# tmbdev/clstm

Measured on AMD Instinct MI355X. Metric: text-line images/sec (fwd+bwd+CTC), 100-unit BiLSTM H=48 T~200, higher is better.
Workload: dtype f32 (operand-exact split): forward, recurrences, CTC, decode in f32 arithmetic; the backward weight-gradient / softmax-backward products take their f32 operands split EXACTLY into three bf16 terms each (x1 + x2 + x3 = x) and sum the six bf16-MFMA products of weight >= 2^-16 in f32 -- what is dropped

## Files before the change

clstm_amd/abi.py:

```python
import ctypes as C
import os

import numpy as np

_HERE = os.path.dirname(os.path.abspath(__file__))
MAX_LAYERS = 4


class NetDesc(C.Structure):
    _fields_ = [("nlayers", C.c_int), ("unidirectional", C.c_int), ("ninput", C.c_int),
                ("nhidden", C.c_int * MAX_LAYERS), ("nclasses", C.c_int)]


class ClstmError(RuntimeError):
    pass


def default_lib_path():
    variant = os.environ.get("CLSTM_HIP_VARIANT", "")
    name = "libclstm_hip_%s.so" % variant if variant else "libclstm_hip.so"
    return os.environ.get("CLSTM_HIP_LIB", os.path.join(_HERE, "lib", name))


_P, _I, _F = C.c_void_p, C.c_int, C.c_float
# ... 91 lines not shown
    "clstm_comm_rank": [_P],
    "clstm_comm_size": [_P],
    "clstm_comm_peer_active": [_P],
    "clstm_comm_peer_capacity": [_P, _P],
    "clstm_allreduce_flat": [_P, _P, C.c_longlong],
    "clstm_net_set_comm": [_P, _P],
    "clstm_net_replica_check": [_P],
    "clstm_net_set_training": [_P, _I],
    "clstm_net_set_overlap": [_P, _I],
    "clstm_net_get_overlap": [_P, _P],
    "clstm_net_set_strict_f32": [_P, _I],
    "clstm_net_overlap_stats": [_P, _P, _P],
    "clstm_debug_lane_ops": [_P],
    "clstm_debug_ctc_cycles": [_P],
    "clstm_debug_gemm": [_I, _P, _P, _P, _I, _I, _I, _I],
    "clstm_debug_path_count": [_I, _P],
    "clstm_debug_set_option": [C.c_char_p, _I],
    "clstm_debug_set_device_error": [_I, _I],
    "clstm_debug_wide_plan": [_P, _P],
    "clstm_debug_net_holds": [_P, _P],
    "clstm_debug_narrow_plan": [_P, _P],
    "clstm_debug_product_plan": [_P, _P],
    "clstm_debug_ctc_plan": [_I, _P, _P, _P, _I, _P, _P],
}
_VALUE_RETURN = {"clstm_net_nparams_for", "clstm_net_nparams", "clstm_abi_version", "clstm_comm_rank", "clstm_comm_size", "clstm_comm_peer_active"}
EXPORTED_SYMBOLS = sorted(list(_SIGS) + ["clstm_last_error", "clstm_abi_version"])
_LATE = {"clstm_debug_net_holds", "clstm_debug_wide_plan", "clstm_debug_narrow_plan", "clstm_debug_product_plan", "clstm_debug_ctc_plan"}


class Lib:

    def __init__(self, path=None):
        path = path or default_lib_path()
        if not os.path.exists(path):
            raise ClstmError(
                "HIP extension not built: %s is missing (no CPU fallback exists; build it with "
                "`make -C clstm_amd/csrc` or __graft_entry__.build())" % path)
        self.path = path
        if os.path.basename(path).startswith("libclstm_hip"):
            try:
                import torch
            except ImportError:
                pass
        self.dll = C.CDLL(path)
        self.dll.clstm_last_error.restype = C.c_char_p
        self.dll.clstm_last_error.argtypes = []
        self.dll.clstm_abi_version.restype = C.c_int
        for name, args in _SIGS.items():
            if (name in _LATE or os.environ.get("CLSTM_ABI_LAX")) and not hasattr(self.dll, name):
                continue
# ... 44 lines not shown
```

clstm_amd/csrc/abi.inc:

```
using namespace clstm;
struct clstm_net {
  std::unique_ptr<size_t> dev_bytes;
  Net net;
  CtcWorkspace ctc;
  DecodeWorkspace dec;
  ScoreWorkspace score;
  BeamWorkspace beam;
};

#define EW(kernel, len, ...) \
  CLSTM_LAUNCH(kernel, dim3(nblocks(len)), dim3(256), 0, g_stream, __VA_ARGS__); check_launch();

struct clstm_charlm { CharLm lm; };
struct clstm_normalizer {
  std::unique_ptr<size_t> dev_bytes;
  Normalizer nz;
};
extern "C" {

const char* clstm_last_error(void) { return g_err.c_str(); }
int clstm_abi_version(void) { return 1; }
int clstm_set_stream(void* s) { g_stream = (hipStream_t)s; return 0; }
int clstm_synchronize(void) { ABI_BEGIN HIPCHECK(hipStreamSynchronize(g_stream)); check_device_errors(); ABI_END }

// ... 768 lines not shown
  static_assert(sizeof(NarrowShape) == 30 * sizeof(int) && sizeof(NarrowPlan) == 11 * sizeof(int), "include/clstm_abi.h documents the int layout");
  NarrowShape h;
  memcpy(&h, shape, sizeof(h));
  REQUIRE(h.pass >= NP_FWD_SAVE && h.pass <= NP_BWD && h.no > 0 && h.ndir >= 1 && h.bs > 0 && h.ncu >= 0, "bad shape");
  const NarrowPlan p = narrow_plan(h);
  memcpy(plan, &p, sizeof(p));
  ABI_END
}
int clstm_debug_product_plan(const int* shape, int* plan) {
  ABI_BEGIN
  REQUIRE(shape && plan, "null argument");
  static_assert(sizeof(ProductShape) == 35 * sizeof(int) && sizeof(ProductPlan) == 39 * sizeof(int), "include/clstm_abi.h documents the int layout");
  ProductShape h;
  memcpy(&h, shape, sizeof(h));
  REQUIRE(h.pass >= PP_FWD && h.pass <= PP_BWD && h.no > 0 && h.ni > 0 && h.ndir >= 1 && h.N > 0 && h.nclasses >= 2 && h.ncu >= 0, "bad shape");
  const ProductPlan p = product_plan(h);
  memcpy(plan, &p, sizeof(p));
  ABI_END
}
int clstm_debug_ctc_plan(int nc, const int* line_off_h, const int* states_h, const int* state_off_h, int bs, int* batch_plan_h,
                         int* line_plan_h) {
  ABI_BEGIN
  describe_ctc_plan(nc, line_off_h, states_h, state_off_h, bs, batch_plan_h, line_plan_h);
  ABI_END
}
int clstm_debug_lane_ops(float* out) {
  ABI_BEGIN
  CLSTM_LAUNCH(k_debug_lane_ops, dim3(1), dim3(64), 0, g_stream, out);
  check_launch();
  ABI_END
}
int clstm_debug_gemm(int mode, const float* A, const float* B, float* Cm, int R, int Cn, int K, int nsplit) {
  ABI_BEGIN
  static thread_local DevBuf<float>* part = nullptr;
  const int sq = gemm_bf16_big(R, Cn) ? GB2_BT : GEMM_BT, kk = gemm_tile256(R, Cn) ? 256 : GB2_BT;
  if (mode == 0) gemm_f32<GEMM_KC, GEMM_MC>(g_stream, gemm_kc(A, K, R, 0), gemm_mc(B, Cn, K, 0), StorePlain{Cm, Cn}, R, Cn, K);
  else if (mode == 1) gemm_f32<GEMM_KC, GEMM_KC>(g_stream, gemm_kc(A, K, R, 0), gemm_kc(B, K, Cn, 0), StorePlain{Cm, Cn}, R, Cn, K);
  else if (mode == 2) {
    if (!part) part = new DevBuf<float>();
    if (nsplit < 1) nsplit = 1;
    part->reserve((size_t)nsplit * R * Cn);
    gemm_f32<GEMM_MC, GEMM_MC>(g_stream, gemm_mc(A, R, K, 0), gemm_mc(B, Cn, K, 0), StorePartial{part->p, R, Cn}, R, Cn, K, nsplit);
    CLSTM_LAUNCH(k_reduce_scatter, dim3(nblocks((size_t)R * Cn)), dim3(256), 0, g_stream,
                 (ReduceDesc{part->p, nullptr, 0LL, nsplit, 1, R, Cn, Cn}), (ReduceDesc{}), Cm, (int*)nullptr, 0, (UpdateFuse{}));
  } else if (mode == 10) gemm_bf16<GEMM_KC, GEMM_MC>(g_stream, gemm_kc(A, K, R, 0), gemm_mc(B, Cn, K, 0), StorePlain{Cm, Cn}, R, Cn, K, sq);
  else if (mode == 11) gemm_bf16<GEMM_KC, GEMM_KC>(g_stream, gemm_kc(A, K, R, 0), gemm_kc(B, K, Cn, 0), StorePlain{Cm, Cn}, R, Cn, K, sq);
// ... 47 lines not shown
```

clstm_amd/csrc/ctc.h:

```cpp
#pragma once
#include <type_traits>
#include "devintrin.h"
#define CR_FN DEVFN
#include "cr_math.h"

namespace clstm {

constexpr int CTC_THREADS = 512;
constexpr int CTC_GROUP = 256;
constexpr int CTC_RMAX = 8;
constexpr int CTC_SMAX_LDS = CTC_GROUP * CTC_RMAX;
constexpr int CTC_MLP = 8;
constexpr int CTC_MLPT = 20;
constexpr int CTC_MAX_TILE = 256;
#ifndef CLSTM_CTC_PD
#define CLSTM_CTC_PD 8
#endif
constexpr int CTC_PD = CLSTM_CTC_PD;
constexpr int CTC_PREG = 34;
constexpr int CTC_NB = 12;
constexpr int CTC_CLANE = 32;
constexpr int CTC_CCACHE = 26;

struct CtcLine { long long lat_off; int b, off, T, soff, S, nu; };
struct CtcArgs {
  const CtcLine* lines;
  const float* P;
  float* Dz;
  float* aligned;
  const int* states;
  float* lat;
  const double* tables;
  int nc;
  int ncp;
  int tile;
  int smax;
  long long* prof;
  int float_logadd;
};

struct CtcLds {
  int tables, part, tot, rowbuf, etile, asum, states, lists, ucol, ucls, ccol, vx, red, dump, words;
};
inline __host__ __device__ CtcLds ctc_lds_layout(int tile, int ncp, int smax) {
  CtcLds l;
  int o = 0;
  l.tables = o; o += CTC_TABLE_WORDS;
  l.part = o;   o += 2 * 512;
  l.tot = o;    o += 2 * smax;
  o = (o + 3) & ~3;
  l.rowbuf = o; o += tile * ncp;
  l.etile = o;  o += tile * (smax | 1);
  l.asum = o;   o += tile;
  l.states = o; o += smax;
  l.lists = o;  o += smax;
  l.ucol = o;   o += smax;
  l.ucls = o;   o += smax;
  l.ccol = o;   o += ncp <= CTC_THREADS + 1 ? ncp : 0;
  l.vx = o;     o += 2 * 2 * (CTC_GROUP + 2);
  l.red = o;    o += 64;
  l.dump = o;   o += 2;
  l.words = o;
  return l;
}
inline __host__ __device__ int ctc_region_words(const CtcLds& l, int tile) { return l.asum + tile - l.rowbuf; }

struct CtcBatchPlan { int tile, smax, ncp, smem; };
inline CtcBatchPlan ctc_batch_plan(int nc, int smax_lines, int tmax) {
  CtcBatchPlan p;
  p.smax = smax_lines < 1 ? 1 : (smax_lines > CTC_SMAX_LDS ? CTC_SMAX_LDS : smax_lines);
  if (tmax < 1) tmax = 1;
  p.ncp = nc | 1;
  const long fixed = (long)ctc_lds_layout(0, p.ncp, p.smax).words * (long)sizeof(float);
  int tile = (int)((160 * 1024 - fixed) / (long)((p.ncp + (p.smax | 1) + 1) * sizeof(float)));
  if (tile > CTC_MAX_TILE) tile = CTC_MAX_TILE;
  if (tile > tmax) tile = tmax;
  p.tile = tile;
  p.smem = (int)((size_t)ctc_lds_layout(tile < 1 ? 1 : tile, p.ncp, p.smax).words * sizeof(float));
  return p;
}
enum CtcForm { CTC_FORM_SHORT = 0, CTC_FORM_TILED = 1, CTC_FORM_HUGE = 2, CTC_FORM_NONE = 3 };
enum CtcRec { CTC_REC_WAVE = 0, CTC_REC_PAIR = 1, CTC_REC_RM2 = 2, CTC_REC_RM8 = 3, CTC_REC_ROUNDS = 4 };
struct CtcLinePlan {
  int form, rec;
  int flat, lds_lat, lanemap;
  int flat_stage, c_in_regs, d_per_state, ntiles;
};
inline __host__ __device__ CtcLinePlan ctc_line_plan(int T, int S, int nu, int nc, int ncp, int tile, int cap) {
  CtcLinePlan p{CTC_FORM_NONE, 0, 0, 0, 0, 0, 0, 0, 0};
  if (T <= 0 || S <= 0) return p;
  const int nub_mk = ((S + 1) / 2 < nc ? (S + 1) / 2 : nc) | 1;
  const int nub = (nu | 1) > nub_mk ? (nu | 1) : nub_mk;
  const bool short_line = T <= CTC_THREADS && (long)T * (ncp + nub) <= cap && (long)T * ((S | 1) + nub) <= cap &&
                          S <= CTC_THREADS && T * S <= CTC_THREADS * CTC_CCACHE && nc <= CTC_THREADS;
  p.form = short_line ? CTC_FORM_SHORT : (S > CTC_SMAX_LDS ? CTC_FORM_HUGE : CTC_FORM_TILED);
  p.rec = S <= 64 ? CTC_REC_WAVE : S <= 128 ? CTC_REC_PAIR : S > CTC_SMAX_LDS ? CTC_REC_ROUNDS
        : (S + CTC_GROUP - 1) / CTC_GROUP <= 2 ? CTC_REC_RM2 : CTC_REC_RM8;
  if (short_line) {
    p.flat = ncp == nc && T * nc <= CTC_PREG * CTC_THREADS;
    p.lds_lat = S <= 64 && 2 * T * S <= cap;
    p.lanemap = S <= 64 && T <= (CTC_THREADS / 64) * CTC_CLANE;
  } else {
    p.flat_stage = ncp == nc;
    p.c_in_regs = (long)T * S <= CTC_THREADS * CTC_CCACHE;
    p.d_per_state = S > CTC_THREADS;
    p.ntiles = (T + tile - 1) / tile;
  }
  return p;
}
inline __host__ __device__ int ctc_scores_behind(int T, int S, int ncp) { return 2 * T * S > T * ncp ? 2 * T * S : T * ncp; }
inline __host__ __device__ bool ctc_scores_in_lds(const CtcLinePlan& p, int T, int S, int ncp, int nu, int cap) {
  return p.lds_lat && ctc_scores_behind(T, S, ncp) + T * (nu | 1) <= cap;
}

DEVFN float ctc_softplus_float(float d) {
  const float L2E_HI = 1.44269502162933349609375f, L2E_LO = 1.92596299112661746e-8f;
  const float t = d * L2E_HI;
  const float r = fmaf(d, L2E_LO, fmaf(d, L2E_HI, -t));
  const float e2 = fast_exp2(t);
  const float ef = fmaf(e2 * 0.693147182464599609375f, r, e2);
  const float sf = ef + 1.0f;
  return fast_log2(sf) * 0.693147182464599609375f;
}
template <bool FLA = false>
DEVFN float ctc_log_add(float x, float y, const CrTables tb) {
  const float d = x - y;
  float lg;
  if constexpr (FLA) lg = ctc_softplus_float(fminf(fmaxf(d, -10.0f), 10.0f)) + y;
  else lg = cr_softplusf(d, tb) + y;
  return fabsf(d) > 10.0f ? fmaxf(x, y) : lg;
}
DEVFN float ctc_limexp(float x) {
  const float xc = fminf(fmaxf(x, -30.0f), 30.0f);
  const float L2E_HI = 1.44269502162933349609375f, L2E_LO = 1.92596299112661746e-8f;
  const float t = xc * L2E_HI;
  const float r = fmaf(xc, L2E_LO, fmaf(xc, L2E_HI, -t));
// ... 175 lines not shown
template <bool FLA = false>
DEVFN void ctc_lattice_huge(const float* lm, float* al, float* be, const CrTables tb, const int T, const int S) {
  const int tid = threadIdx.x;
  const int grp = tid >> 8, u = tid & (CTC_GROUP - 1);
  const bool rev = grp == 1;
  const size_t latbytes = (size_t)T * S * 4;
  const BufF32 lmb = make_buf(lm, latbytes), outb = make_buf(rev ? be : al, latbytes);
  auto loff = [&](int i, int j) -> unsigned {
    return (unsigned)(rev ? (size_t)(T - 1 - i) * S + (S - 1 - j) : (size_t)i * S + j) * 4u;
  };
  __syncthreads();
  for (int i = 0; i < T; i++) {
    for (int j = u; j < S; j += CTC_GROUP) {
      const float lmv = buf_load(lmb, loff(i, j));
      const float vj = i == 0 ? (float)(-5.0 * j) : buf_load_wt(outb, loff(i - 1, j));
      const float w = j == 0 ? (float)(-5.0 * i) : (i == 0 ? (float)(-5.0 * (j - 1)) : buf_load_wt(outb, loff(i - 1, j - 1)));
      buf_store_wt(outb, loff(i, j), ctc_log_add<FLA>(vj + lmv, w + lmv, tb));
    }
    drain_vmem();
    __syncthreads();
  }
}

#define CTC_STAMP(k) do { if (a.prof && b == 0 && threadIdx.x == 0) a.prof[k] = dev_clock(); } while (0)
constexpr int CTC_TREG = (CTC_TABLE_DOUBLES + CTC_THREADS - 1) / CTC_THREADS;

template <bool FLA>
DEVFN void ctc_short_line(const CtcArgs& a, float* lds, const CtcLds& L, const CrTables tb, const int b, float* lm,
                          const int off, const int T, const int S, const double (&treg)[CTC_TREG],
                          const float (&preg)[CTC_PREG], const CtcLinePlan& pl) {
  const int tid = threadIdx.x, lane = tid & 63, wave = wave_uniform(tid >> 6);
  const int nc = a.nc, ncp = a.ncp;
  double* part = reinterpret_cast<double*>(lds + L.part);
  double* tot = reinterpret_cast<double*>(lds + L.tot);
  float* rowbuf = lds + L.rowbuf;
  float* etile = rowbuf;
  const int cap = ctc_region_words(L, a.tile);
  const bool flat = pl.flat;
  int* stl = reinterpret_cast<int*>(lds + L.states);
  int* lists = reinterpret_cast<int*>(lds + L.lists);
  int* ucol = reinterpret_cast<int*>(lds + L.ucol);
  int* ucls = reinterpret_cast<int*>(lds + L.ucls);
  int* ccol = reinterpret_cast<int*>(lds + L.ccol);
  float* red = lds + L.red;
  int* wcnt = reinterpret_cast<int*>(red + 16);
  float* dump = lds + L.dump;
  float* al = lm + (size_t)T * S;
  float* be = al + (size_t)T * S;
  const int TS = T * S, sp = S | 1;
  const size_t latbytes = (size_t)TS * 4;
  const BufF32 pb = make_buf(a.P + (size_t)off * nc, (size_t)T * nc * 4);

  const int npost = T * nc;

  int* firstof = reinterpret_cast<int*>(rowbuf);
// ... 20 lines not shown
  for (int w = 0; w < CTC_THREADS / 64; w++) {
    const int cP = wcnt[w * 4], cB = wcnt[w * 4 + 1], cL = wcnt[w * 4 + 2], cR = wcnt[w * 4 + 3];
    const bool pre = w < wave;
    bP += pre ? cP : 0; bB += pre ? cB : 0; bL += pre ? cL : 0; bR += pre ? cR : 0;
    nu += cP; nb += cB; nf += cL;
  }
  const int nr = S - nb - nf, nup = nu | 1;
  if (tid < nc) {
    const int r = bP + __builtin_popcountll(mP & below);
    ccol[tid] = pres ? r : -1;
    if (pres) ucls[r] = tid;
  }
  if (isblank) lists[bB + __builtin_popcountll(mB & below)] = tid;
  if (islab) lists[nb + bL + __builtin_popcountll(mL & below)] = tid;
  if (isrep) lists[nb + nf + bR + __builtin_popcountll(mR & below)] = tid;
  __syncthreads();
  if (live) ucol[tid] = ccol[sc];
  CTC_STAMP(12);
  const bool lds_lat = pl.lds_lat;
  const bool lm_lds = ctc_scores_in_lds(pl, T, S, ncp, nu, cap);
  float* lmu = rowbuf + (lm_lds ? ctc_scores_behind(T, S, ncp) : T * ncp);
  float pw[CTC_NB];
  {
    const int n = T * nu;
    const int dq = CTC_THREADS / nu, dr = CTC_THREADS - dq * nu;
    int tq = tid / nu, uq = tid - tq * nu;
#pragma unroll
    for (int u = 0; u < CTC_NB; u++) {
      const bool in = tid + u * CTC_THREADS < n;
      pw[u] = buf_load(pb, in ? (unsigned)(tq * nc + ucls[in ? uq : 0]) * 4u : BUF_OOB);
      tq += dq; uq += dr;
      if (uq >= nu) { uq -= nu; tq++; }
    }
  }
  {
    double* tabs = reinterpret_cast<double*>(lds + L.tables);
#pragma unroll
    for (int k = 0; k < CTC_TREG; k++)
      if (tid + k * CTC_THREADS < CTC_TABLE_DOUBLES) tabs[tid + k * CTC_THREADS] = treg[k];
  }

  if (flat) {
#pragma unroll
    for (int k = 0; k < CTC_PREG; k++) {
      const int i = tid + k * CTC_THREADS;
      float* w = i < npost ? &rowbuf[i] : dump;
      *w = fmaxf(1e-5f, preg[k]);
    }
  } else {
// ... 75 lines not shown
#pragma unroll
        for (int u = 0; u < 8; u++) {
          const int t = t0 + u * (CTC_THREADS / 64);
          buf_store(lmw, (sok && t < T) ? (unsigned)(t * S + st) * 4u : BUF_OOB, x[u]);
        }
      }
    }
  }
  CTC_STAMP(1);

  float* all = rowbuf;
  float* bel = rowbuf + TS;
  if (lm_lds) ctc_lattice<true, true, FLA>(lm, all, bel, lds + L.vx, dump, tb, T, S, pl.rec, lmu, nup, ucol);
  else if (lds_lat) ctc_lattice<true, false, FLA>(lm, all, bel, lds + L.vx, dump, tb, T, S, pl.rec);
  else ctc_lattice<false, false, FLA, CTC_REC_RM2>(lm, al, be, lds + L.vx, dump, tb, T, S, pl.rec);
  const BufF32 dzb = make_buf(a.Dz + (size_t)off * nc, (size_t)T * nc * 4);
  const BufF32 agb = make_buf(a.aligned ? a.aligned + (size_t)off * nc : a.Dz, a.aligned ? (size_t)T * nc * 4 : 0);
  const bool one_wave = pl.rec == CTC_REC_WAVE;
  if (!one_wave || (wave & 2)) {
    const int w0 = !one_wave ? wave : (wave & 1) + ((wave >> 2) << 1), nw = !one_wave ? CTC_THREADS / 64 : 4;
    for (int cb = 0; cb < nc; cb += 64) {
      const int c = cb + lane;
      const bool absent = c < nc && ccol[c < nc ? c : 0] < 0;
      for (int t0 = w0; t0 < T; t0 += 8 * nw) {
        float x[8];
        unsigned ofs[8];
#pragma unroll
        for (int u = 0; u < 8; u++) {
          const int t = t0 + u * nw;
          ofs[u] = (absent && t < T) ? (unsigned)(t * nc + c) * 4u : BUF_OOB;
          x[u] = buf_load(pb, ofs[u]);
        }
#pragma unroll
        for (int u = 0; u < 8; u++) {
          buf_store(agb, ofs[u], 0.0f);
          buf_store(dzb, ofs[u], 0.0f - x[u]);
        }
      }
    }
  }
  __syncthreads();
  CTC_STAMP(2);

  const bool lanemap = pl.lanemap;
  if (lanemap) {
    const BufF32 alb = make_buf(al, latbytes), beb = make_buf(be, latbytes);
    const bool sok = lane < S;
    const int sl = sok ? lane : 0;
    float bo[CTC_CLANE];
    float mx = -3.0e38f;
    auto load_cells = [&](auto lds_tag) {
      constexpr bool LL = decltype(lds_tag)::value;
#pragma unroll
// ... 33 lines not shown
    for (int g = 0; g < CTC_CLANE / 4; g++) {
      if (wave + 32 * g < T) {
#pragma unroll
        for (int u = 0; u < 4; u++) {
          const int k = 4 * g + u, t = wave + 8 * k;
          const float e = ctc_limexp(bo[k] - mx);
          bo[k] = e;
          acc += (t < T) ? (double)e : 0.0;
        }
      }
    }
    CTC_STAMP(3);
    if (sok) part[wave * S + lane] = acc;
    __syncthreads();
    CTC_STAMP(8);
    if (tid < S) {
      double sum = 0.0;
      for (int k = 0; k < CTC_THREADS / 64; k++) sum += part[k * S + tid];
      tot[tid] = 1.0 / fmax(1e-9, sum);
    }
    __syncthreads();
    CTC_STAMP(9);
    const double it = tot[sl];
#pragma unroll
    for (int g = 0; g < CTC_CLANE / 4; g++) {
      if (wave + 32 * g < T) {
#pragma unroll
        for (int u = 0; u < 4; u++) {
          const int k = 4 * g + u, t = wave + 8 * k;
          float* w = (sok && t < T) ? &etile[t * sp + lane] : dump;
          *w = (float)((double)bo[k] * it);
        }
      }
    }
    __syncthreads();
    CTC_STAMP(4);
  } else {
  {
    const BufF32 alb = make_buf(al, latbytes), beb = make_buf(be, latbytes);
    float bo[CTC_CCACHE];
    float mx = -3.0e38f;
    if (lds_lat) {
#pragma unroll
      for (int k = 0; k < CTC_CCACHE; k++) {
        const int i = tid + k * CTC_THREADS;
        const int ic = i < TS ? i : 0;
        bo[k] = i < TS ? all[ic] + bel[ic] : -3.0e38f;
        mx = fmaxf(mx, bo[k]);
      }
    } else {
#pragma unroll
      for (int k = 0; k < CTC_CCACHE; k++) {
        const int i = tid + k * CTC_THREADS;
// ... 46 lines not shown
    if (act) part[q * S + st] = acc;
    __syncthreads();
    CTC_STAMP(8);
    if (tid < S) {
      double sum = 0.0;
      for (int k = 0; k < Q; k++) sum += part[k * S + tid];
      tot[tid] = 1.0 / fmax(1e-9, sum);
    }
    __syncthreads();
    CTC_STAMP(9);
  }
  CTC_STAMP(4);
  }

  float* rowc = rowbuf + T * sp;
  auto project = [&](auto pre_tag) {
    constexpr bool PRE = decltype(pre_tag)::value;
    if (wave >= 4) {
      for (int f0 = 0; f0 < nf; f0 += 64) {
        const bool fok = f0 + lane < nf;
        const int st = lists[nb + (fok ? f0 + lane : 0)];
        const int col = ucol[st];
        const double it = PRE ? 1.0 : tot[st];
        int t0 = wave - 4;
        for (; t0 + 28 < T; t0 += 4 * 8) {
          float x[8];
#pragma unroll
          for (int u = 0; u < 8; u++) x[u] = etile[(t0 + 4 * u) * sp + st];
#pragma unroll
          for (int u = 0; u < 8; u++) {
            float* w = fok ? &rowc[(t0 + 4 * u) * nup + col] : dump;
            *w = PRE ? x[u] : (float)((double)x[u] * it);
          }
        }
        if (t0 < T) {
          float x[8];
#pragma unroll
          for (int u = 0; u < 8; u++) { const int t = t0 + 4 * u; x[u] = etile[(t < T ? t : T - 1) * sp + st]; }
#pragma unroll
          for (int u = 0; u < 8; u++) {
            const int t = t0 + 4 * u;
            float* w = (fok && t < T) ? &rowc[t * nup + col] : dump;
            *w = PRE ? x[u] : (float)((double)x[u] * it);
          }
        }
      }
    } else {
      for (int t = tid; t < T; t += 256) {
        const float* e = etile + t * sp;
        double blank = 0.0;
        int i0 = 0;
        for (; i0 + 8 <= nb; i0 += 8) {
          float x[8];
          double it[8];
#pragma unroll
          for (int u = 0; u < 8; u++) {
            const int st = lists[i0 + u];
            x[u] = e[st];
            it[u] = PRE ? 1.0 : tot[st];
          }
#pragma unroll
          for (int u = 0; u < 8; u++) blank += PRE ? (double)x[u] : (double)(float)((double)x[u] * it[u]);
        }
        if (i0 < nb) {
          float x[8];
          double it[8];
#pragma unroll
          for (int u = 0; u < 8; u++) {
            const int st = lists[i0 + u < nb ? i0 + u : 0];
            x[u] = e[st];
            it[u] = PRE ? 1.0 : tot[st];
          }
#pragma unroll
          for (int u = 0; u < 8; u++) blank += (i0 + u < nb) ? (PRE ? (double)x[u] : (double)(float)((double)x[u] * it[u])) : 0.0;
        }
        part[t] = blank;
      }
    }
  };
  if (lanemap) project(std::true_type{}); else project(std::false_type{});
  __syncthreads();
  CTC_STAMP(10);
  for (int t = tid; t < T; t += CTC_THREADS) {
    float* row = rowc + t * nup;
    const float* e = etile + t * sp;
    for (int i = 0; i < nr; i++) {
      const int st = lists[nb + nf + i];
      row[ucol[st]] += lanemap ? e[st] : (float)((double)e[st] * tot[st]);
    }
    if (nb > 0) row[ccol[0]] = (float)part[t];
    double total = 0.0;
    int u0 = 0;
    for (; u0 + 8 <= nu; u0 += 8) {
      float x[8];
#pragma unroll
      for (int u = 0; u < 8; u++) x[u] = row[u0 + u];
#pragma unroll
      for (int u = 0; u < 8; u++) total += (double)x[u];
    }
    if (u0 < nu) {
      float x[8];
#pragma unroll
      for (int u = 0; u < 8; u++) x[u] = row[u0 + u < nu ? u0 + u : 0];
#pragma unroll
      for (int u = 0; u < 8; u++) total += (u0 + u < nu) ? (double)x[u] : 0.0;
    }
    part[t] = 1.0 / fmax(total, 1e-9);
  }
  __syncthreads();
  CTC_STAMP(11);
  {
    const int n = T * nu;
    const int dq = CTC_THREADS / nu, dr = CTC_THREADS - dq * nu;
    int tq = tid / nu, uq = tid - tq * nu;
    for (int i0 = tid; i0 < n; i0 += CTC_NB * CTC_THREADS) {
      float p[CTC_NB], av[CTC_NB];
      unsigned ofs[CTC_NB];
#pragma unroll
      for (int u = 0; u < CTC_NB; u++) {
        const bool in = i0 + u * CTC_THREADS < n;
        const int tc = in ? tq : 0, uc = in ? uq : 0;
        ofs[u] = in ? (unsigned)(tc * nc + ucls[uc]) * 4u : BUF_OOB;
        av[u] = (float)((double)rowc[tc * nup + uc] * part[tc]);
        tq += dq; uq += dr;
        if (uq >= nu) { uq -= nu; tq++; }
      }
      if (i0 == tid) {
#pragma unroll
        for (int u = 0; u < CTC_NB; u++) p[u] = pw[u];
      } else {
#pragma unroll
        for (int u = 0; u < CTC_NB; u++) p[u] = buf_load(pb, ofs[u]);
      }
#pragma unroll
      for (int u = 0; u < CTC_NB; u++) {
        buf_store(agb, ofs[u], av[u]);
        buf_store(dzb, ofs[u], av[u] - p[u]);
      }
    }
  }
  CTC_STAMP(5);
}

template <bool FLA>
__global__ __launch_bounds__(CTC_THREADS) void ctc_align_kernel(CtcArgs a) {
  float* lds = dyn_smem<float>();
  const CtcLds L = ctc_lds_layout(a.tile, a.ncp, a.smax);
  double* tabs = reinterpret_cast<double*>(lds + L.tables);
  double* part = reinterpret_cast<double*>(lds + L.part);
  double* tot = reinterpret_cast<double*>(lds + L.tot);
  float* rowbuf = lds + L.rowbuf;
  float* etile = lds + L.etile;
  float* asum = lds + L.asum;
  int* stl = reinterpret_cast<int*>(lds + L.states);
  float* vx = lds + L.vx;
  float* red = lds + L.red;
  const CrTables tb{tabs, tabs + 32, tabs + 96, tabs + 160};
  const int tid = threadIdx.x, lane = tid & 63, wave = wave_uniform(tid >> 6);
  const CtcLine ln = a.lines[blockIdx.x];
  const int b = ln.b;
  const int nc = a.nc, ncp = a.ncp, TT = a.tile;
  const int off = ln.off, T = ln.T;
  const int soff = ln.soff, S = ln.S;
  const CtcLinePlan pl = ctc_line_plan(T, S, ln.nu, nc, ncp, TT, ctc_region_words(L, TT));
  if (pl.form == CTC_FORM_NONE) return;
  const float* P = a.P + (size_t)off * nc;
  float* Dz = a.Dz + (size_t)off * nc;
  float* lm = a.lat + ln.lat_off;
  float* al = lm + (size_t)T * S;
  float* be = al + (size_t)T * S;
  CTC_STAMP(0);
  const bool short_line = pl.form == CTC_FORM_SHORT;
  const int st0 = a.states[soff + (tid < S ? tid : 0)];
  double treg[CTC_TREG];
#pragma unroll
  for (int k = 0; k < CTC_TREG; k++) {
    const int i = tid + k * CTC_THREADS;
    treg[k] = a.tables[i < CTC_TABLE_DOUBLES ? i : CTC_TABLE_DOUBLES - 1];
  }
  if (short_line) {
    const BufF32 pb = make_buf(P, (size_t)T * nc * 4);
    float preg[CTC_PREG];
    if (pl.flat) {
#pragma unroll
      for (int k = 0; k < CTC_PREG; k++) preg[k] = buf_load(pb, (unsigned)(tid + k * CTC_THREADS) * 4u);
    }
    if (tid < S) stl[tid] = st0;
    for (int s = tid + CTC_THREADS; s < S; s += CTC_THREADS) stl[s] = a.states[soff + s];
    __syncthreads();
    ctc_short_line<FLA>(a, lds, L, tb, b, lm, off, T, S, treg, preg, pl);
    return;
  }
  const bool huge = pl.form == CTC_FORM_HUGE;
  const int* stg = a.states + soff;
  double* totg = reinterpret_cast<double*>(lm + (((size_t)3 * T * S + 1) & ~(size_t)1));
  if (!huge) {
    if (tid < S) stl[tid] = st0;
    for (int s = tid + CTC_THREADS; s < S; s += CTC_THREADS) stl[s] = a.states[soff + s];
  }
  auto state_at = [&](int s) -> int { return huge ? stg[s] : stl[s]; };
  int* lists = reinterpret_cast<int*>(lds + L.lists);
  int nblank = 0;
  if (!huge) {
    __syncthreads();
    int* cnt = reinterpret_cast<int*>(red + 32);
    if (wave == 0) {
      int nb = 0;
      for (int s0 = 0; s0 < S; s0 += 64) nb += __builtin_popcountll(wave_ballot(s0 + lane < S && stl[s0 + lane < S ? s0 + lane : 0] == 0));
      int ib = 0, il = nb;
      const unsigned long long below = (1ull << lane) - 1ull;
      for (int s0 = 0; s0 < S; s0 += 64) {
        const bool in = s0 + lane < S;
        const bool isb = in && stl[in ? s0 + lane : 0] == 0;
// ... 328 lines not shown
```

clstm_amd/csrc/ctc_run.inc:

```
static thread_local long long* g_last_ctc_prof = nullptr;
struct CtcWorkspace {
  CtcArgs pending{};
  size_t pending_smem = 0;
  int pending_bs = 0;
  PinnedRing ring;
  DevBuf<long long> prof;
  DevBuf<double> tables;
  DevBuf<char> meta;
  DevBuf<float> lat;
  std::vector<int> nu, seen;
};
static void upload_ctc_tables(DevBuf<double>& tables) {
  if (tables.p) return;
  tables.reserve(CTC_TABLE_DOUBLES);
  std::vector<double> tb(CTC_TABLE_DOUBLES);
  for (int i = 0; i < 32; i++) tb[i] = CTC_EXP2_32[i];
  for (int i = 0; i < 64; i++) { tb[32 + i] = CTC_LOG_INVC[i]; tb[96 + i] = CTC_LOG_LOGC[i]; }
  for (int k = 0; k < 2 * CTC_SP_KMAX + 1; k++)
    for (int c = 0; c < 4; c++) tb[160 + 4 * k + c] = CTC_SOFTPLUS[k][c];
  HIPCHECK(hipMemcpy(tables.p, tb.data(), CTC_TABLE_DOUBLES * sizeof(double), hipMemcpyHostToDevice));
}
static void launch_ctc_align(const CtcWorkspace& w, hipStream_t s) {
  if (!w.pending.float_logadd) CLSTM_LAUNCH(ctc_align_kernel<false>, dim3(w.pending_bs), dim3(CTC_THREADS), w.pending_smem, s, w.pending);
  else CLSTM_LAUNCH(ctc_align_kernel<true>, dim3(w.pending_bs), dim3(CTC_THREADS), w.pending_smem, s, w.pending);
  check_launch();
}
static void expand_transcripts(const int* labels_h, const int* L_h, int n, std::vector<int>& states, std::vector<int>& soff) {
  soff.assign(n + 1, 0);
  int lpos = 0;
  for (int b = 0; b < n; b++) {
    const int L = L_h[b];
    REQUIRE(L >= 0, "negative transcript length");
    states.resize(soff[b] + 2 * L + 1);
    clstm_mktargets(states.data() + soff[b], labels_h + lpos, L);
    for (int i = 0; i < L; i++) REQUIRE(labels_h[lpos + i] != 0, "transcript contains the blank class (Codec::encode asserts c != 0, clstm.cc:232)");
    lpos += L;
    soff[b + 1] = soff[b] + 2 * L + 1;
  }
}
static void check_target_classes(int nc, const int* states_h, int ns) {
  for (int i = 0; i < ns; i++) REQUIRE(states_h[i] >= 0 && states_h[i] < nc, "target class out of range");
}
static CtcBatchPlan ctc_minibatch_plan(int nc, const int* line_off_h, const int* state_off_h, int bs) {
  int smax = 1, tmax = 1;
  for (int b = 0; b < bs; b++) {
    smax = std::max(smax, state_off_h[b + 1] - state_off_h[b]);
    tmax = std::max(tmax, line_off_h[b + 1] - line_off_h[b]);
  }
  const CtcBatchPlan bp = ctc_batch_plan(nc, smax, tmax);
  REQUIRE(bp.tile >= 1, "too many classes / target states for the CTC row tile");
  REQUIRE(bp.smem <= 160 * 1024, "CTC LDS carve exceeds 160 KiB");
  return bp;
}
static void ctc_distinct_classes(int nc, const int* states_h, const int* state_off_h, int bs, std::vector<int>& nu, std::vector<int>& seen) {
  nu.assign(bs, 0);
  seen.assign(nc, -1);
  for (int b = 0; b < bs; b++)
    for (int i = state_off_h[b]; i < state_off_h[b + 1]; i++)
      if (seen[states_h[i]] != b) { seen[states_h[i]] = b; nu[b]++; }
}
constexpr int CTC_PLAN_INTS = 13;
static void describe_ctc_plan(int nc, const int* line_off_h, const int* states_h, const int* state_off_h, int bs, int* batch_plan_h,
                              int* line_plan_h) {
  REQUIRE(bs > 0 && nc >= 1 && line_off_h && states_h && state_off_h && batch_plan_h && line_plan_h, "empty batch / null argument");
  for (int b = 0; b < bs; b++)
    REQUIRE(line_off_h[b + 1] >= line_off_h[b] && state_off_h[b + 1] >= state_off_h[b], "bad offsets");
  check_target_classes(nc, states_h, state_off_h[bs]);
  const CtcBatchPlan bp = ctc_minibatch_plan(nc, line_off_h, state_off_h, bs);
  batch_plan_h[0] = bp.tile; batch_plan_h[1] = bp.smax; batch_plan_h[2] = bp.ncp; batch_plan_h[3] = bp.smem;
  const int cap = ctc_region_words(ctc_lds_layout(bp.tile, bp.ncp, bp.smax), bp.tile);
  std::vector<int> nus, seen;
  ctc_distinct_classes(nc, states_h, state_off_h, bs, nus, seen);
// ... 28 lines not shown
  {
    char* stage = (char*)w.ring.acquire(nln + nst);
    std::vector<int> order(bs);
    for (int b = 0; b < bs; b++) order[b] = b;
    std::stable_sort(order.begin(), order.end(), [&](int x, int y) { return lo[x + 1] - lo[x] > lo[y + 1] - lo[y]; });
    CtcLine* ln = (CtcLine*)stage;
    for (int i = 0; i < bs; i++) {
      const int b = order[i];
      ln[i] = CtcLine{lo[b], b, line_off_h[b], line_off_h[b + 1] - line_off_h[b], state_off_h[b], state_off_h[b + 1] - state_off_h[b], nus[b]};
    }
    if (ns > 0) memcpy(stage + nln, states_h, (size_t)ns * sizeof(int));
    if (defer) {
      defer->src = (const int*)stage; defer->dst = (int*)w.meta.p; defer->nwords = (int)((nln + nst) / sizeof(int));
    } else {
      HIPCHECK(hipMemcpyAsync(w.meta.p, stage, nln + nst, hipMemcpyHostToDevice, s));
      w.ring.commit(s);
    }
  }
  CtcArgs a{};
  a.lines = (const CtcLine*)w.meta.p;
  a.P = probs; a.Dz = deltas; a.aligned = aligned;
  a.states = (const int*)(w.meta.p + nln);
  a.lat = w.lat.p; a.nc = nc;
  w.prof.reserve(16); a.prof = w.prof.p; g_last_ctc_prof = w.prof.p;
  a.float_logadd = dbg_opt("ctc_float") != 0;
  upload_ctc_tables(w.tables);
  a.tables = w.tables.p;
  const CtcBatchPlan bp = ctc_minibatch_plan(nc, line_off_h, state_off_h, bs);
  a.smax = bp.smax; a.ncp = bp.ncp; a.tile = bp.tile;
  const size_t smem = (size_t)bp.smem;
#ifndef CLSTM_HIP_EMU
  static size_t smem_set = 0;
  if (smem > smem_set) {
    HIPCHECK(hipFuncSetAttribute((const void*)ctc_align_kernel<false>, hipFuncAttributeMaxDynamicSharedMemorySize, (int)smem));
    HIPCHECK(hipFuncSetAttribute((const void*)ctc_align_kernel<true>, hipFuncAttributeMaxDynamicSharedMemorySize, (int)smem));
    smem_set = smem;
  }
#endif
  w.pending = a; w.pending_smem = smem; w.pending_bs = bs;
  if (launch) launch_ctc_align(w, s);
}
struct DecodeWorkspace {
  DevBuf<int> line_off, idx;
  DevBuf<float> val;
  DevBuf<int> out;
  PinnedBuf<int> host;
};
static void run_decode(DecodeWorkspace& w, const float* probs, int nc, const int* line_off_h, int bs,
                       int* classes_h, int* locs_h, int* counts_h, hipStream_t s, float* conf_h = nullptr) {
  const int N = line_off_h[bs];
  REQUIRE(bs > 0 && N > 0, "empty batch");
  const size_t nout = (size_t)bs + 3 * (size_t)N;
// ... 308 lines not shown
```

clstm_amd/csrc/dbgopt.h:

```cpp
#pragma once
#include <cstdlib>
#include <cstring>
#include <map>
#include <stdexcept>
#include <string>

namespace clstm {
struct DbgOptDef { const char* name; int dflt; };
inline constexpr DbgOptDef DBG_OPTS[] = {
    {"gemm_stag", 2},
    {"bwd_c32", 1},
    {"rec_x3", 1},
    {"pack_tiles", 1},
    {"fuse_wx", 1},
    {"gemm_b16mc", 1},
    {"dw_x3", 1},
    {"gemm_x3", 1},
    {"split_terms", 3},
    {"xd_prologue", 2},
    {"fwd_mfma", 1},
    {"bwd_mfma", 1},
    {"bwd_mfma_fused", 1},
    {"ctc_float", 0},
    {"peer_two_phase", 1},
};
inline const DbgOptDef* dbg_opt_def(const char* name) {
  for (const DbgOptDef& o : DBG_OPTS)
    if (strcmp(o.name, name) == 0) return &o;
  return nullptr;
}
inline std::map<std::string, int>& dbg_opts() {
  static std::map<std::string, int> m = [] {
    std::map<std::string, int> r;
    const char* e = getenv("CLSTM_DEBUG");
    if (e) {
      std::string s(e);
      size_t i = 0;
      while (i < s.size()) {
        size_t j = s.find(',', i);
        if (j == std::string::npos) j = s.size();
        const std::string kv = s.substr(i, j - i);
        const size_t eq = kv.find('=');
        if (!kv.empty()) {
          const std::string name = kv.substr(0, eq);
          if (eq == std::string::npos || !dbg_opt_def(name.c_str()))
            throw std::runtime_error("CLSTM_DEBUG: unknown option '" + name + "' (clstm_amd/csrc/dbgopt.h lists them as name=value)");
// ... 18 lines not shown
```

include/clstm_abi.h:

```cpp
#ifndef CLSTM_ABI_H_
#define CLSTM_ABI_H_

#include <stddef.h>
#ifdef __cplusplus
extern "C" {
#endif

enum { CLSTM_LIN = 0, CLSTM_SIG = 1, CLSTM_TANH = 2, CLSTM_RELU = 3, CLSTM_LOGMAG = 4 };

const char* clstm_last_error(void);
int clstm_abi_version(void);
int clstm_set_stream(void* hip_stream);
int clstm_synchronize(void);

int clstm_forward_nonlin0(float* y_v, int len, int nl);
int clstm_backward_nonlin0(const float* y_v, float* y_d, int len, int nl);
int clstm_forward_nonlin(float* y_v, const float* x_v, int len, int nl);
int clstm_backward_nonlin(const float* y_v, const float* y_d, float* x_d, int len, int nl);
int clstm_forward_lin1(float* y_v, const float* W_v, const float* x_v, int n, int m, int bs);
int clstm_backward_lin1(const float* y_d, const float* W_v, float* W_d, const float* x_v, float* x_d,
                        int n, int m, int bs);
int clstm_forward_full1(float* y_v, const float* W_v, const float* x_v, int n, int m, int bs, int nl);
int clstm_backward_full1(const float* y_v, float* y_d, const float* W_v, float* W_d, const float* x_v,
                         float* x_d, int n, int m, int bs, int nl);
// ... 125 lines not shown
int clstm_comm_create(clstm_comm** out, const char* id_h, int rank, int nranks);
int clstm_comm_destroy(clstm_comm* comm);
int clstm_comm_rank(clstm_comm* comm);
int clstm_comm_size(clstm_comm* comm);
int clstm_comm_peer_active(clstm_comm* comm);
int clstm_comm_peer_capacity(clstm_comm* comm, long long* floats);
int clstm_allreduce_flat(clstm_comm* comm, float* buf_d, long long n);
int clstm_net_set_comm(clstm_net* net, clstm_comm* comm);
int clstm_net_replica_check(clstm_net* net);
int clstm_net_set_training(clstm_net* net, int on);

int clstm_debug_lane_ops(float* out);
int clstm_debug_ctc_cycles(long long* out_h);
int clstm_debug_gemm(int mode, const float* A, const float* B, float* C, int R, int Cn, int K, int nsplit);
int clstm_debug_path_count(int which, long long* out_h);
int clstm_debug_set_option(const char* name, int value);
int clstm_debug_set_device_error(int which, int value);
int clstm_debug_wide_plan(const int* shape, int* plan);
int clstm_debug_net_holds(clstm_net* net, int* out);
int clstm_debug_narrow_plan(const int* shape, int* plan);
int clstm_debug_product_plan(const int* shape, int* plan);
int clstm_debug_ctc_plan(int nc, const int* line_off_h, const int* states_h, const int* state_off_h, int bs, int* batch_plan_h,
                         int* line_plan_h);

#ifdef __cplusplus
}
#endif
#endif
```

Before: 232,600.

## Split CTC short-line output phase across multiple blocks per line when CUs idle

Launches up to four blocks per text line for the CTC align kernel when the batch is small relative to the CU count. Each block redoes the full forward-backward pass but writes only its own slice of time frames in the projection and delta-output phases. A smaller unroll width is also used for the output loop when the slice is short. This aims to fill idle CUs and shorten the output-writing tail, at the cost of redundant alpha/beta recursion per part and a larger grid.

Result: faster. 235,100 (median of 6 runs) (+1.1%).

```diff
diff --git a/clstm_amd/abi.py b/clstm_amd/abi.py
--- a/clstm_amd/abi.py
+++ b/clstm_amd/abi.py
@@ -137,10 +137,14 @@
     "clstm_debug_narrow_plan": [_P, _P],
     "clstm_debug_product_plan": [_P, _P],
     "clstm_debug_ctc_plan": [_I, _P, _P, _P, _I, _P, _P],
+    "clstm_debug_ctc_split": [_I, _I, _P],
+    "clstm_debug_ctc_part_frames": [_I, _I, _I, _P],
+    "clstm_debug_ctc_cycles_part": [_I, _P],
 }
 _VALUE_RETURN = {"clstm_net_nparams_for", "clstm_net_nparams", "clstm_abi_version", "clstm_comm_rank", "clstm_comm_size", "clstm_comm_peer_active"}
 EXPORTED_SYMBOLS = sorted(list(_SIGS) + ["clstm_last_error", "clstm_abi_version"])
-_LATE = {"clstm_debug_net_holds", "clstm_debug_wide_plan", "clstm_debug_narrow_plan", "clstm_debug_product_plan", "clstm_debug_ctc_plan"}
+_LATE = {"clstm_debug_net_holds", "clstm_debug_wide_plan", "clstm_debug_narrow_plan", "clstm_debug_product_plan", "clstm_debug_ctc_plan",
+         "clstm_debug_ctc_split", "clstm_debug_ctc_part_frames", "clstm_debug_ctc_cycles_part"}
 
 
 class Lib:
diff --git a/clstm_amd/csrc/abi.inc b/clstm_amd/csrc/abi.inc
--- a/clstm_amd/csrc/abi.inc
+++ b/clstm_amd/csrc/abi.inc
@@ -814,6 +814,29 @@
                          int* line_plan_h) {
   ABI_BEGIN
   describe_ctc_plan(nc, line_off_h, states_h, state_off_h, bs, batch_plan_h, line_plan_h);
+  ABI_END
+}
+int clstm_debug_ctc_split(int bs, int ncu, int* nsplit_h) {
+  ABI_BEGIN
+  REQUIRE(bs > 0 && ncu >= 0 && nsplit_h, "bad argument");
+  const int opt = dbg_opt("ctc_split");
+  REQUIRE(opt == 0 || opt == 1 || opt == 2 || opt == 4, "option ctc_split must be 0, 1, 2 or 4");
+  *nsplit_h = ctc_nsplit(bs, ncu > 0 ? ncu : device_cu_count(), opt);
+  ABI_END
+}
+int clstm_debug_ctc_part_frames(int T, int n, int k, int* range_h) {
+  ABI_BEGIN
+  REQUIRE(T >= 0 && n >= 1 && k >= 0 && k < n && range_h, "bad argument");
+  const CtcFrames f = ctc_part_frames(T, n, k);
+  range_h[0] = f.lo; range_h[1] = f.hi;
+  ABI_END
+}
+int clstm_debug_ctc_cycles_part(int part, long long* out_h) {
+  ABI_BEGIN
+  REQUIRE(g_last_ctc_prof, "no CTC launch yet");
+  REQUIRE(part >= 0 && part < 4 && out_h, "bad argument");
+  HIPCHECK(hipStreamSynchronize(g_stream));
+  HIPCHECK(hipMemcpy(out_h, g_last_ctc_prof + 16 * part, 16 * sizeof(long long), hipMemcpyDeviceToHost));
   ABI_END
 }
 int clstm_debug_lane_ops(float* out) {
diff --git a/clstm_amd/csrc/ctc.h b/clstm_amd/csrc/ctc.h
--- a/clstm_amd/csrc/ctc.h
+++ b/clstm_amd/csrc/ctc.h
@@ -19,6 +19,7 @@
 constexpr int CTC_PD = CLSTM_CTC_PD;
 constexpr int CTC_PREG = 34;
 constexpr int CTC_NB = 12;
+constexpr int CTC_NBS = 4;
 constexpr int CTC_CLANE = 32;
 constexpr int CTC_CCACHE = 26;
 
@@ -37,6 +38,8 @@
   int smax;
   long long* prof;
   int float_logadd;
+  int bs;
+  int nsplit;
 };
 
 struct CtcLds {
@@ -65,9 +68,22 @@
 }
 inline __host__ __device__ int ctc_region_words(const CtcLds& l, int tile) { return l.asum + tile - l.rowbuf; }
 
-struct CtcBatchPlan { int tile, smax, ncp, smem; };
-inline CtcBatchPlan ctc_batch_plan(int nc, int smax_lines, int tmax) {
+struct CtcBatchPlan { int tile, smax, ncp, smem, nsplit; };
+inline int ctc_nsplit(int bs, int ncu, int opt) {
+  if (opt == 1 || opt == 2 || opt == 4) return opt;
+  for (int n = 4; n > 1; n >>= 1)
+    if ((long)bs * n <= ncu) return n;
+  return 1;
+}
+struct CtcFrames { int lo, hi; };
+inline __host__ __device__ CtcFrames ctc_part_frames(int T, int n, int k) {
+  const int c = (T + n - 1) / n;
+  const int lo = k * c < T ? k * c : T, hi = (k + 1) * c < T ? (k + 1) * c : T;
+  return CtcFrames{lo, hi};
+}
+inline CtcBatchPlan ctc_batch_plan(int nc, int smax_lines, int tmax, int bs = 1, int ncu = 0, int split_opt = 1) {
   CtcBatchPlan p;
+  p.nsplit = ctc_nsplit(bs, ncu, split_opt);
   p.smax = smax_lines < 1 ? 1 : (smax_lines > CTC_SMAX_LDS ? CTC_SMAX_LDS : smax_lines);
   if (tmax < 1) tmax = 1;
   p.ncp = nc | 1;
@@ -112,6 +128,9 @@
 inline __host__ __device__ bool ctc_scores_in_lds(const CtcLinePlan& p, int T, int S, int ncp, int nu, int cap) {
   return p.lds_lat && ctc_scores_behind(T, S, ncp) + T * (nu | 1) <= cap;
 }
+inline __host__ __device__ bool ctc_line_splits(const CtcLinePlan& p, int T, int S, int ncp, int nu, int cap) {
+  return p.form == CTC_FORM_SHORT && ctc_scores_in_lds(p, T, S, ncp, nu, cap);
+}
 
 DEVFN float ctc_softplus_float(float d) {
   const float L2E_HI = 1.44269502162933349609375f, L2E_LO = 1.92596299112661746e-8f;
@@ -333,15 +352,17 @@
   }
 }
 
-#define CTC_STAMP(k) do { if (a.prof && b == 0 && threadIdx.x == 0) a.prof[k] = dev_clock(); } while (0)
+#define CTC_STAMP(k) do { if (a.prof && b == 0 && threadIdx.x == 0) a.prof[16 * ipart + (k)] = dev_clock(); } while (0)
 constexpr int CTC_TREG = (CTC_TABLE_DOUBLES + CTC_THREADS - 1) / CTC_THREADS;
 
 template <bool FLA>
 DEVFN void ctc_short_line(const CtcArgs& a, float* lds, const CtcLds& L, const CrTables tb, const int b, float* lm,
                           const int off, const int T, const int S, const double (&treg)[CTC_TREG],
-                          const float (&preg)[CTC_PREG], const CtcLinePlan& pl) {
+                          const float (&preg)[CTC_PREG], const CtcLinePlan& pl, const int ipart, const int nparts) {
   const int tid = threadIdx.x, lane = tid & 63, wave = wave_uniform(tid >> 6);
   const int nc = a.nc, ncp = a.ncp;
+  const CtcFrames fr = ctc_part_frames(T, nparts, ipart);
+  const int t_lo = fr.lo, t_hi = fr.hi;
   double* part = reinterpret_cast<double*>(lds + L.part);
   double* tot = reinterpret_cast<double*>(lds + L.tot);
   float* rowbuf = lds + L.rowbuf;
@@ -408,9 +429,10 @@
   float* lmu = rowbuf + (lm_lds ? ctc_scores_behind(T, S, ncp) : T * ncp);
   float pw[CTC_NB];
   {
-    const int n = T * nu;
+    const int n = (t_hi - t_lo) * nu;
     const int dq = CTC_THREADS / nu, dr = CTC_THREADS - dq * nu;
     int tq = tid / nu, uq = tid - tq * nu;
+    tq += t_lo;
 #pragma unroll
     for (int u = 0; u < CTC_NB; u++) {
       const bool in = tid + u * CTC_THREADS < n;
@@ -532,13 +554,13 @@
     for (int cb = 0; cb < nc; cb += 64) {
       const int c = cb + lane;
       const bool absent = c < nc && ccol[c < nc ? c : 0] < 0;
-      for (int t0 = w0; t0 < T; t0 += 8 * nw) {
+      for (int t0 = t_lo + w0; t0 < t_hi; t0 += 8 * nw) {
         float x[8];
         unsigned ofs[8];
 #pragma unroll
         for (int u = 0; u < 8; u++) {
           const int t = t0 + u * nw;
-          ofs[u] = (absent && t < T) ? (unsigned)(t * nc + c) * 4u : BUF_OOB;
+          ofs[u] = (absent && t < t_hi) ? (unsigned)(t * nc + c) * 4u : BUF_OOB;
           x[u] = buf_load(pb, ofs[u]);
         }
 #pragma unroll
@@ -618,13 +640,15 @@
     __syncthreads();
     CTC_STAMP(9);
     const double it = tot[sl];
+    const int k_lo = (t_lo - wave + 7) >> 3, k_hi = (t_hi - wave + 7) >> 3;
+    const unsigned cells = (unsigned)(((1ull << k_hi) - 1ull) & ~((1ull << k_lo) - 1ull));
 #pragma unroll
     for (int g = 0; g < CTC_CLANE / 4; g++) {
-      if (wave + 32 * g < T) {
+      if ((cells >> (4 * g)) & 0xFu) {
 #pragma unroll
         for (int u = 0; u < 4; u++) {
           const int k = 4 * g + u, t = wave + 8 * k;
-          float* w = (sok && t < T) ? &etile[t * sp + lane] : dump;
+          float* w = (sok && ((cells >> k) & 1u)) ? &etile[t * sp + lane] : dump;
           *w = (float)((double)bo[k] * it);
         }
       }
@@ -717,8 +741,8 @@
         const int st = lists[nb + (fok ? f0 + lane : 0)];
         const int col = ucol[st];
         const double it = PRE ? 1.0 : tot[st];
-        int t0 = wave - 4;
-        for (; t0 + 28 < T; t0 += 4 * 8) {
+        int t0 = t_lo + wave - 4;
+        for (; t0 + 28 < t_hi; t0 += 4 * 8) {
           float x[8];
 #pragma unroll
           for (int u = 0; u < 8; u++) x[u] = etile[(t0 + 4 * u) * sp + st];
@@ -728,20 +752,20 @@
             *w = PRE ? x[u] : (float)((double)x[u] * it);
           }
         }
-        if (t0 < T) {
+        if (t0 < t_hi) {
           float x[8];
 #pragma unroll
-          for (int u = 0; u < 8; u++) { const int t = t0 + 4 * u; x[u] = etile[(t < T ? t : T - 1) * sp + st]; }
+          for (int u = 0; u < 8; u++) { const int t = t0 + 4 * u; x[u] = etile[(t < t_hi ? t : t_hi - 1) * sp + st]; }
 #pragma unroll
           for (int u = 0; u < 8; u++) {
             const int t = t0 + 4 * u;
-            float* w = (fok && t < T) ? &rowc[t * nup + col] : dump;
+            float* w = (fok && t < t_hi) ? &rowc[t * nup + col] : dump;
             *w = PRE ? x[u] : (float)((double)x[u] * it);
           }
         }
       }
     } else {
-      for (int t = tid; t < T; t += 256) {
+      for (int t = t_lo + tid; t < t_hi; t += 256) {
         const float* e = etile + t * sp;
         double blank = 0.0;
         int i0 = 0;
@@ -776,7 +800,7 @@
   if (lanemap) project(std::true_type{}); else project(std::false_type{});
   __syncthreads();
   CTC_STAMP(10);
-  for (int t = tid; t < T; t += CTC_THREADS) {
+  for (int t = t_lo + tid; t < t_hi; t += CTC_THREADS) {
     float* row = rowc + t * nup;
     const float* e = etile + t * sp;
     for (int i = 0; i < nr; i++) {
@@ -804,15 +828,17 @@
   }
   __syncthreads();
   CTC_STAMP(11);
-  {
-    const int n = T * nu;
+  auto write_out = [&](auto nb_tag) {
+    constexpr int NB = decltype(nb_tag)::value;
+    const int n = (t_hi - t_lo) * nu;
     const int dq = CTC_THREADS / nu, dr = CTC_THREADS - dq * nu;
     int tq = tid / nu, uq = tid - tq * nu;
-    for (int i0 = tid; i0 < n; i0 += CTC_NB * CTC_THREADS) {
-      float p[CTC_NB], av[CTC_NB];
-      unsigned ofs[CTC_NB];
-#pragma unroll
-      for (int u = 0; u < CTC_NB; u++) {
+    tq += t_lo;
+    for (int i0 = tid; i0 < n; i0 += NB * CTC_THREADS) {
+      float p[NB], av[NB];
+      unsigned ofs[NB];
+#pragma unroll
+      for (int u = 0; u < NB; u++) {
         const bool in = i0 + u * CTC_THREADS < n;
         const int tc = in ? tq : 0, uc = in ? uq : 0;
         ofs[u] = in ? (unsigned)(tc * nc + ucls[uc]) * 4u : BUF_OOB;
@@ -822,18 +848,20 @@
       }
       if (i0 == tid) {
 #pragma unroll
-        for (int u = 0; u < CTC_NB; u++) p[u] = pw[u];
+        for (int u = 0; u < NB; u++) p[u] = pw[u];
       } else {
 #pragma unroll
-        for (int u = 0; u < CTC_NB; u++) p[u] = buf_load(pb, ofs[u]);
-      }
-#pragma unroll
-      for (int u = 0; u < CTC_NB; u++) {
+        for (int u = 0; u < NB; u++) p[u] = buf_load(pb, ofs[u]);
+      }
+#pragma unroll
+      for (int u = 0; u < NB; u++) {
         buf_store(agb, ofs[u], av[u]);
         buf_store(dzb, ofs[u], av[u] - p[u]);
       }
     }
-  }
+  };
+  if ((t_hi - t_lo) * nu <= CTC_NBS * CTC_THREADS) write_out(std::integral_constant<int, CTC_NBS>{});
+  else write_out(std::integral_constant<int, CTC_NB>{});
   CTC_STAMP(5);
 }
 
@@ -852,13 +880,16 @@
   float* red = lds + L.red;
   const CrTables tb{tabs, tabs + 32, tabs + 96, tabs + 160};
   const int tid = threadIdx.x, lane = tid & 63, wave = wave_uniform(tid >> 6);
-  const CtcLine ln = a.lines[blockIdx.x];
+  const int ipart = a.nsplit > 1 ? (int)blockIdx.x / a.bs : 0;
+  const CtcLine ln = a.lines[(int)blockIdx.x - ipart * a.bs];
   const int b = ln.b;
   const int nc = a.nc, ncp = a.ncp, TT = a.tile;
   const int off = ln.off, T = ln.T;
   const int soff = ln.soff, S = ln.S;
   const CtcLinePlan pl = ctc_line_plan(T, S, ln.nu, nc, ncp, TT, ctc_region_words(L, TT));
   if (pl.form == CTC_FORM_NONE) return;
+  const int nparts = a.nsplit > 1 && ctc_line_splits(pl, T, S, ncp, ln.nu, ctc_region_words(L, TT)) ? a.nsplit : 1;
+  if (ipart >= nparts) return;
   const float* P = a.P + (size_t)off * nc;
   float* Dz = a.Dz + (size_t)off * nc;
   float* lm = a.lat + ln.lat_off;
@@ -883,7 +914,7 @@
     if (tid < S) stl[tid] = st0;
     for (int s = tid + CTC_THREADS; s < S; s += CTC_THREADS) stl[s] = a.states[soff + s];
     __syncthreads();
-    ctc_short_line<FLA>(a, lds, L, tb, b, lm, off, T, S, treg, preg, pl);
+    ctc_short_line<FLA>(a, lds, L, tb, b, lm, off, T, S, treg, preg, pl, ipart, nparts);
     return;
   }
   const bool huge = pl.form == CTC_FORM_HUGE;
diff --git a/clstm_amd/csrc/ctc_run.inc b/clstm_amd/csrc/ctc_run.inc
--- a/clstm_amd/csrc/ctc_run.inc
+++ b/clstm_amd/csrc/ctc_run.inc
@@ -21,8 +21,9 @@
   HIPCHECK(hipMemcpy(tables.p, tb.data(), CTC_TABLE_DOUBLES * sizeof(double), hipMemcpyHostToDevice));
 }
 static void launch_ctc_align(const CtcWorkspace& w, hipStream_t s) {
-  if (!w.pending.float_logadd) CLSTM_LAUNCH(ctc_align_kernel<false>, dim3(w.pending_bs), dim3(CTC_THREADS), w.pending_smem, s, w.pending);
-  else CLSTM_LAUNCH(ctc_align_kernel<true>, dim3(w.pending_bs), dim3(CTC_THREADS), w.pending_smem, s, w.pending);
+  const dim3 grid((unsigned)w.pending_bs * (unsigned)w.pending.nsplit);
+  if (!w.pending.float_logadd) CLSTM_LAUNCH(ctc_align_kernel<false>, grid, dim3(CTC_THREADS), w.pending_smem, s, w.pending);
+  else CLSTM_LAUNCH(ctc_align_kernel<true>, grid, dim3(CTC_THREADS), w.pending_smem, s, w.pending);
   check_launch();
 }
 static void expand_transcripts(const int* labels_h, const int* L_h, int n, std::vector<int>& states, std::vector<int>& soff) {
@@ -41,13 +42,14 @@
 static void check_target_classes(int nc, const int* states_h, int ns) {
   for (int i = 0; i < ns; i++) REQUIRE(states_h[i] >= 0 && states_h[i] < nc, "target class out of range");
 }
-static CtcBatchPlan ctc_minibatch_plan(int nc, const int* line_off_h, const int* state_off_h, int bs) {
+static CtcBatchPlan ctc_minibatch_plan(int nc, const int* line_off_h, const int* state_off_h, int bs, int ncu = 0, int split_opt = 1) {
   int smax = 1, tmax = 1;
   for (int b = 0; b < bs; b++) {
     smax = std::max(smax, state_off_h[b + 1] - state_off_h[b]);
     tmax = std::max(tmax, line_off_h[b + 1] - line_off_h[b]);
   }
-  const CtcBatchPlan bp = ctc_batch_plan(nc, smax, tmax);
+  REQUIRE(split_opt == 0 || split_opt == 1 || split_opt == 2 || split_opt == 4, "option ctc_split must be 0, 1, 2 or 4");
+  const CtcBatchPlan bp = ctc_batch_plan(nc, smax, tmax, bs, ncu, split_opt);
   REQUIRE(bp.tile >= 1, "too many classes / target states for the CTC row tile");
   REQUIRE(bp.smem <= 160 * 1024, "CTC LDS carve exceeds 160 KiB");
   return bp;
@@ -122,12 +124,24 @@
   a.P = probs; a.Dz = deltas; a.aligned = aligned;
   a.states = (const int*)(w.meta.p + nln);
   a.lat = w.lat.p; a.nc = nc;
-  w.prof.reserve(16); a.prof = w.prof.p; g_last_ctc_prof = w.prof.p;
+  w.prof.reserve(16 * 4); a.prof = w.prof.p; g_last_ctc_prof = w.prof.p;
   a.float_logadd = dbg_opt("ctc_float") != 0;
   upload_ctc_tables(w.tables);
   a.tables = w.tables.p;
-  const CtcBatchPlan bp = ctc_minibatch_plan(nc, line_off_h, state_off_h, bs);
+  const CtcBatchPlan bp = ctc_minibatch_plan(nc, line_off_h, state_off_h, bs, device_cu_count(), dbg_opt("ctc_split"));
   a.smax = bp.smax; a.ncp = bp.ncp; a.tile = bp.tile;
+  a.bs = bs; a.nsplit = bp.nsplit;
+  if (a.nsplit > 1) {
+    const int cap = ctc_region_words(ctc_lds_layout(bp.tile, bp.ncp, bp.smax), bp.tile);
+    bool any = false;
+    for (int b = 0; b < bs && !any; b++) {
+      const int T = line_off_h[b + 1] - line_off_h[b], S = state_off_h[b + 1] - state_off_h[b];
+      any = ctc_line_splits(ctc_line_plan(T, S, nus[b], nc, bp.ncp, bp.tile, cap), T, S, bp.ncp, nus[b], cap);
+    }
+    const uintptr_t p0 = (uintptr_t)probs, p1 = p0 + (size_t)line_off_h[bs] * nc * sizeof(float);
+    auto overlaps = [&](const float* o) { return o && (uintptr_t)o < p1 && (uintptr_t)o + (p1 - p0) > p0; };
+    if (!any || overlaps(deltas) || overlaps(aligned)) a.nsplit = 1;
+  }
   const size_t smem = (size_t)bp.smem;
 #ifndef CLSTM_HIP_EMU
   static size_t smem_set = 0;
diff --git a/clstm_amd/csrc/dbgopt.h b/clstm_amd/csrc/dbgopt.h
--- a/clstm_amd/csrc/dbgopt.h
+++ b/clstm_amd/csrc/dbgopt.h
@@ -22,6 +22,7 @@
     {"bwd_mfma", 1},
     {"bwd_mfma_fused", 1},
     {"ctc_float", 0},
+    {"ctc_split", 0},
     {"peer_two_phase", 1},
 };
 inline const DbgOptDef* dbg_opt_def(const char* name) {
diff --git a/include/clstm_abi.h b/include/clstm_abi.h
--- a/include/clstm_abi.h
+++ b/include/clstm_abi.h
@@ -171,6 +171,9 @@
 int clstm_debug_product_plan(const int* shape, int* plan);
 int clstm_debug_ctc_plan(int nc, const int* line_off_h, const int* states_h, const int* state_off_h, int bs, int* batch_plan_h,
                          int* line_plan_h);
+int clstm_debug_ctc_split(int bs, int ncu, int* nsplit_h);
+int clstm_debug_ctc_part_frames(int T, int n, int k, int* range_h);
+int clstm_debug_ctc_cycles_part(int part, long long* out_h);
 
 #ifdef __cplusplus
 }
```
